# quadram-institute-bioscience/tatajuba

Measured on AMD Instinct MI355X. Metric: reads/s (whole node), 150 bp synthetic FASTQ, homopolymer scan + context histogram, higher is better.
Workload: dtype u8/u64

## Files before the change

tatajuba_amd/csrc/hopo_device.hip:

```cpp

#include <hip/hip_runtime.h>
#include <rccl/rccl.h>
#include <dlfcn.h>
#include <mutex>
#include <string>
#include <new>
#include <stdint.h>
#include <stdio.h>
#include <stdlib.h>
#include <string.h>
#include <stdarg.h>
#include <limits.h>
#include <float.h>
#include <algorithm>
#include <vector>
#include <memory>

#include "../../include/tatajuba_amd.h"
#include "../../include/tatajuba_variants.h"
#include "../../include/tatajuba_features.h"
#include "../../include/tatajuba_effects.h"
#include "../../include/tatajuba_sites.h"
#include "../../include/tatajuba_depths.h"
#include "../../include/tatajuba_distances.h"
// ... 1267 lines not shown
__device__ __noinline__ u64 fast_general_tract (const FastLds &T, const uint8_t *__restrict__ seq, long n_bytes, long g0, int s, int k, int mprime, bool n_tile)
{
  u64 c0, c1; u32 base, len10, flag;
  if (!fast_tract<true> (T, seq, n_bytes, g0, s, k, mprime, c0, c1, base, len10, flag, n_tile)) return 0ull;
  return pack_rec1 ((u32) c0, (u32) c1, base, len10, flag);
}

__device__ __forceinline__ void lds_dma32 (const uint8_t *sbase, u32 voff, void *lds_wave_base)
{
  const u32 m0v = (u32) (size_t) (lptr_t) lds_wave_base;
  asm volatile ("s_nop 0\n\tglobal_load_lds_dwordx4 %0, %1\n\tglobal_load_lds_dwordx4 %0, %1 offset:1024"
                :: "v"(voff), "s"(sbase), "{m0}"(m0v) : "memory");
}

template <int W, bool LOG = false>
__global__ __launch_bounds__ (FK_BLOCK, FK_BLOCK * (LOG ? FK_LOG_WG_PER_CU : FK_WG_PER_CU) / 256)
void scan_fast_kernel (const uint8_t *__restrict__ seq, long n_bytes, long n_ftiles, int k, int mprime,
                       Buckets BK, DevCounters *ctr, u32 *__restrict__ slow_list, int par, int all_slow, LogSpace LG)
{
  static_assert (!LOG || W <= 2, "the record log holds one-word and two-word records");
  __shared__ FastLds T;
  __shared__ uint4 raw[FK_WIN / 16];
  __shared__ std::conditional_t<LOG, LogLds, StageLds<W, true>> SL;
  auto make_sink = [&] () {
    if constexpr (LOG) return LogSink<W> {SL, LG, ctr, k, 0u, 0u, 0u, 0u, 0ull};
    else return StageSink<W, FK_BLOCK, true> {SL, BK, ctr, k, 0u, 0u, 0u};
  };
  auto sink = make_sink ();
  sink.start ();

  const int tid = threadIdx.x, lane = tid & 63;
// ... 1313 lines not shown
__global__ __launch_bounds__ (256)
void bin_count_kernel (const u64 *__restrict__ in, long n, int k, int nbits, u32 *__restrict__ bins, uint4 *__restrict__ cov, long cov_vec, int grouped,
                       const FinPlan *__restrict__ plan = nullptr)
{
  if (plan) { if (!plan->ok) return; n = plan->n1; nbits = plan->nbits; cov_vec = plan->t / 2; }
  for (long i = (long) blockIdx.x * 256 + threadIdx.x; i < cov_vec; i += (long) gridDim.x * 256) cov[i] = make_uint4 (0, 0, 0, 0);
  for (long i0 = (long) blockIdx.x * 256; i0 < n; i0 += (long) gridDim.x * 256) {
    const long i = i0 + threadIdx.x;
    u32 bin = 0;
    if (i < n) { const u64 *p = in + 3 * i; bin = bin_of_record (p[0], p[1], p[2], k, nbits); }
    (void) bin_reserve (bins, bin, i < n, grouped);
  }
}

#define BS_MAXBINS (1 << BS_MAXBITS)
#define WGS_CHUNK  16384

#define WGS_PAD(i) ((i) + ((i) >> 5))
struct WgScanLds { u32 a[WGS_CHUNK + WGS_CHUNK / 32 + 1]; u32 wsum[16]; u32 vmax; };

__device__ __forceinline__ u32 wg_exclusive_scan (const u32 *__restrict__ in, int n_all, u32 *__restrict__ out, u32 *__restrict__ out2, WgScanLds &L, u32 &vmax)
{
  const int tid = threadIdx.x, lane = tid & 63, wave = tid >> 6;
  if (tid == 0) L.vmax = 0;
  u32 carry = 0;
  for (int base = 0; base < n_all; base += WGS_CHUNK) {
    const int n = min (WGS_CHUNK, n_all - base);
    const int per = (n + 1023) / 1024;
    for (int i = tid; i < n; i += 1024) L.a[WGS_PAD (i)] = in[base + i];
    __syncthreads ();
    u32 sum = 0, mx = 0;
    for (int j = 0; j < per; j++) { const int b = tid * per + j; if (b < n) { const u32 v = L.a[WGS_PAD (b)]; sum += v; mx = max (mx, v); } }
    const u32 incl = wave_inclusive_scan (sum);
    if (lane == 63) L.wsum[wave] = incl;
    for (int o = 32; o > 0; o >>= 1) mx = max (mx, (u32) __shfl_down ((int) mx, o));
    if (lane == 0 && mx) atomicMax (&L.vmax, mx);
    __syncthreads ();
    u32 run = carry + incl - sum, total = 0;
    for (int w = 0; w < 16; w++) { const u32 x = L.wsum[w]; if (w < wave) run += x; total += x; }
    for (int j = 0; j < per; j++) { const int b = tid * per + j; if (b < n) { const u32 v = L.a[WGS_PAD (b)]; L.a[WGS_PAD (b)] = run; run += v; } }
    __syncthreads ();
    for (int i = tid; i < n; i += 1024) { const u32 v = L.a[WGS_PAD (i)]; out[base + i] = v; if (out2) out2[base + i] = v; }
    carry += total;
    __syncthreads ();
  }
  vmax = L.vmax;
  return carry;
}

__global__ __launch_bounds__ (1024)
void bin_scan_kernel (u32 *__restrict__ bins, int nbins, u32 *__restrict__ binstart, u32 rank_max, FinCounts *fin, const FinPlan *__restrict__ plan = nullptr)
{
  __shared__ WgScanLds L;
  u32 vmax;
  if (plan) { if (!plan->ok) return; nbins = plan->nbins; }
  const u32 total = wg_exclusive_scan (bins, nbins, binstart, bins, L, vmax);
  if (threadIdx.x == 0) { binstart[nbins] = total; fin->sort_fallback = vmax > rank_max ? 1u : 0u; }
}

__global__ __launch_bounds__ (256)
void bin_scatter_kernel (const u64 *__restrict__ in, u64 *__restrict__ out, long n, int k, int nbits, u32 *__restrict__ cursors,
                         const FinPlan *__restrict__ plan = nullptr, uint4 *__restrict__ cov = nullptr)
{
  if (plan) { if (!plan->ok) return; n = plan->n1; nbits = plan->nbits; }
  if (cov) for (long i = (long) blockIdx.x * 256 + threadIdx.x; i < plan->t / 2; i += (long) gridDim.x * 256) cov[i] = make_uint4 (0, 0, 0, 0);
  for (long i = (long) blockIdx.x * 256 + threadIdx.x; i < n; i += (long) gridDim.x * 256) {
    const u64 *p = in + 3 * i;
    const u64 a = p[0], b = p[1], m = p[2];
    u64 *q = out + 3 * (u64) atomicAdd (&cursors[bin_of_record (a, b, m, k, nbits)], 1u);
    q[0] = a; q[1] = b; q[2] = m;
  }
}
// ... 183 lines not shown
  if ((threadIdx.x & 63) == 0) s_best[threadIdx.x >> 6] = best;
  __syncthreads ();
  if (threadIdx.x == 0) {
    for (int w = 1; w < (int) blockDim.x / 64; w++) best = max (best, s_best[w]);
    if (best != INT_MIN) atomicMax (result, best);
  }
}

__global__ __launch_bounds__ (256)
void cov_max_kernel (const u64 *__restrict__ tab, long t, int *result)
{
  __shared__ int s_best[4];
  cov_max_part (tab, t, result, s_best);
}

#define BSI_WAVES 1

template <int J>
__device__ __forceinline__ u32 lane_xor (u32 v, int lane)
{
  if constexpr (J == 1) return (u32) __builtin_amdgcn_update_dpp (0, (int) v, 0xB1, 0xF, 0xF, false);
  else if constexpr (J == 2) return (u32) __builtin_amdgcn_update_dpp (0, (int) v, 0x4E, 0xF, 0xF, false);
  else if constexpr (J == 4 || J == 8) {
    const u32 up = (u32) __builtin_amdgcn_update_dpp (0, (int) v, 0x100 + J, 0xF, 0xF, false);
    const u32 dn = (u32) __builtin_amdgcn_update_dpp (0, (int) v, 0x110 + J, 0xF, 0xF, false);
    return (lane & J) ? dn : up;
  }
  else if constexpr (J == 16) { const auto r = __builtin_amdgcn_permlane16_swap (v, v, false, false); return (lane & 16) ? r[0] : r[1]; }
  else { const auto r = __builtin_amdgcn_permlane32_swap (v, v, false, false); return (lane & 32) ? r[0] : r[1]; }
}

__global__ __launch_bounds__ (64 * BSI_WAVES)
void bin_sort_index_kernel (const u64 *__restrict__ in, u64 *__restrict__ out, const u32 *__restrict__ binstart, int nbins, const FinCounts *fin,
                            int min_coverage, u64 *__restrict__ cov_tab, int log2t,
                            u32 *__restrict__ binctx, u32 *__restrict__ tstart, u32 *__restrict__ tend, const FinPlan *__restrict__ plan = nullptr,
                            int cov_direct = 0)
{
  __shared__ alignas (16) u32 hd[BSI_WAVES][BS_RANK_MAX];
  __shared__ u32 sz[BSI_WAVES][BS_RANK_MAX];
  const int lane = threadIdx.x & 63, wave = threadIdx.x >> 6;
  const int bin0 = (int) blockIdx.x * BSI_WAVES + wave;
  u32 st0 = 0, en0 = 0;
  if (bin0 < nbins) { st0 = binstart[bin0]; en0 = binstart[bin0 + 1]; }
  if (plan) { if (!plan->ok) return; nbins = plan->nbins; log2t = plan->log2t; cov_direct = (int) plan->cov_direct; }
  if (fin->sort_fallback) return;
  u32 *H = hd[wave], *E = sz[wave];
  for (int bin = bin0; bin < nbins; bin += gridDim.x * BSI_WAVES) {
    const u32 st = (bin == bin0) ? st0 : binstart[bin], s = ((bin == bin0) ? en0 : binstart[bin + 1]) - st;
    if (s == 0) { if (lane == 0) binctx[bin] = 0; continue; }
    const u64 *R = in + 3 * (u64) st;
    u32 nkeep = 0;
    if (s <= 64u) {
      const bool valid = (u32) lane < s;
      u64 a0 = 0, a1 = 0, am = 0;
      if (valid) { a0 = R[3 * lane]; a1 = R[3 * lane + 1]; am = R[3 * lane + 2]; }
      const int w = meta_count (am);
      u64 cas_a = 0, cas_b = 0;
      if (!cov_direct && valid) cov_add2_issue ((u32) (a0 & 0x7FFFFFFFull), (u32) (a1 & 0x7FFFFFFFull), w, cov_tab, log2t, cas_a, cas_b);
      u32 kh = valid ? 2u | ((u32) am & 1u) : 0u;
      u32 kl = ((((u32) (am >> TJ_META_LEN_SHIFT) & 0x3FFu) ^ 0x200u) << 6) | (63u - (u32) lane);
      u32 x0 = (u32) a0, x1 = (u32) (a0 >> 32), y0 = (u32) a1, y1 = (u32) (a1 >> 32), m0 = (u32) am, m1 = (u32) (am >> 32);
      auto step = [&] (auto jc, int kk) {
        constexpr int J = decltype (jc)::value;
        const u32 ox0 = lane_xor<J> (x0, lane), ox1 = lane_xor<J> (x1, lane), oy0 = lane_xor<J> (y0, lane), oy1 = lane_xor<J> (y1, lane);
        const u32 om0 = lane_xor<J> (m0, lane), om1 = lane_xor<J> (m1, lane), okh = lane_xor<J> (kh, lane), okl = lane_xor<J> (kl, lane);
        const u64 mx = ((u64) x1 << 32) | x0, my = ((u64) y1 << 32) | y0, ox = ((u64) ox1 << 32) | ox0, oy = ((u64) oy1 << 32) | oy0;
        const bool mine_first = (kh > okh) | ((kh == okh) & ((mx > ox) | ((mx == ox) & ((my > oy) | ((my == oy) & (kl > okl))))));
        const bool want_first = ((lane & kk) == 0) == ((lane & J) == 0);
        const bool take = mine_first != want_first;
        x0 = take ? ox0 : x0; x1 = take ? ox1 : x1; y0 = take ? oy0 : y0; y1 = take ? oy1 : y1;
        m0 = take ? om0 : m0; m1 = take ? om1 : m1; kh = take ? okh : kh; kl = take ? okl : kl;
      };
#pragma unroll
// ... 20 lines not shown
      const u32 last_incl = (u32) __builtin_amdgcn_ds_bpermute ((int) ((next_head - 1u) << 2), (int) incl);
      const int depth = (int) (last_incl - (incl - (u32) cnt));
      const bool keep = head & (depth >= min_coverage);
      const u64 keeps = __ballot (keep);
      if (keep) {
        const u32 o = (u32) __popcll (keeps & ((1ull << lane) - 1ull));
        tstart[st + o] = st + (u32) lane;
        tend[st + o] = st + next_head;
      }
      nkeep = (u32) __popcll (keeps);
      if (cov_direct) {
        if (head) { cov_direct_add ((u32) (b0 & 0x7FFFFFFFull), depth, cov_tab); cov_direct_add ((u32) (b1 & 0x7FFFFFFFull), depth, cov_tab); }
      }
      else if (valid) {
        asm volatile ("" : "+v"(cas_a), "+v"(cas_b));
        cov_add2_finish ((u32) (a0 & 0x7FFFFFFFull), (u32) (a1 & 0x7FFFFFFFull), w, cov_tab, log2t, cas_a, cas_b);
      }
      if (lane == 0) binctx[bin] = nkeep;
      asm volatile ("s_waitcnt lgkmcnt(0)" ::: "memory");
      __builtin_amdgcn_wave_barrier ();
      continue;
    }
    for (u32 t0 = 0; t0 < s; t0 += 64) {
      const u32 t = t0 + lane;
      bool keep = false;
      if (t < s) {
        const u64 a0 = R[3 * t], a1 = R[3 * t + 1], am = R[3 * t + 2];
        u32 rank = 0, ctx_before = 0, ctx_size = 0;
        int depth = 0;
        const u32 abase = (u32) am & 1u, alen = ((u32) (am >> TJ_META_LEN_SHIFT) & 0x3FFu) ^ 0x200u;
        for (u32 j0 = 0; j0 < s; j0 += 4) {
// ... 41 lines not shown
          o += ((g.x & 0x80000000u) && (g.x & 0x7FFFFFFFu) < rank) ? 1u : 0u;
          o += (j + 1u < s && (g.y & 0x80000000u) && (g.y & 0x7FFFFFFFu) < rank) ? 1u : 0u;
          o += (j + 2u < s && (g.z & 0x80000000u) && (g.z & 0x7FFFFFFFu) < rank) ? 1u : 0u;
          o += (j + 3u < s && (g.w & 0x80000000u) && (g.w & 0x7FFFFFFFu) < rank) ? 1u : 0u;
        }
        tstart[st + o] = st + rank;
        tend[st + o] = st + rank + E[t];
      }
    }
    if (lane == 0) binctx[bin] = nkeep;
    asm volatile ("s_waitcnt lgkmcnt(0)" ::: "memory");
    __builtin_amdgcn_wave_barrier ();
  }
}

__global__ __launch_bounds__ (1024)
void bin_ctx_scan_kernel (const u32 *__restrict__ binctx, int nbins, u32 *__restrict__ binout, FinCounts *fin, const FinPlan *__restrict__ plan = nullptr)
{
  __shared__ WgScanLds L;
  u32 vmax;
  if (plan) { if (!plan->ok) return; nbins = plan->nbins; }
  const u32 total = wg_exclusive_scan (binctx, nbins, binout, nullptr, L, vmax);
  if (threadIdx.x == 0 && !fin->sort_fallback) { fin->n_idx = total; fin->coverage = INT_MIN; }
}

__global__ __launch_bounds__ (256)
void bin_ctx_write_kernel (const u32 *__restrict__ binstart, const u32 *__restrict__ binctx, const u32 *__restrict__ binout, int nbins,
                           const u32 *__restrict__ tstart, const u32 *__restrict__ tend, int *__restrict__ idx_initial, int *__restrict__ idx_final,
                           const u64 *__restrict__ cov_tab, long t, FinCounts *fin, const FinPlan *__restrict__ plan = nullptr)
{
  __shared__ int s_best[4];
  if (plan) { if (!plan->ok) return; nbins = plan->nbins; t = plan->t; }
  if (fin->sort_fallback) return;
  const int lane = threadIdx.x & 63, wave = threadIdx.x >> 6;
  for (int bin = blockIdx.x * 4 + wave; bin < nbins; bin += gridDim.x * 4) {
    const u32 cnt = binctx[bin], st = binstart[bin], o0 = binout[bin];
    for (u32 o = lane; o < cnt; o += 64) { idx_initial[o0 + o] = (int) tstart[st + o]; idx_final[o0 + o] = (int) tend[st + o]; }
  }
  cov_max_part (cov_tab, t, &fin->coverage, s_best);
}

#define MG_RANK_MAX 256
#define TJ_META_SAMPLE_SHIFT 52

__global__ __launch_bounds__ (256)
void merge_scatter_kernel (const u64 *__restrict__ in, u64 *__restrict__ out, long n, int k, int nbits, u32 *__restrict__ cursors,
                           const long *__restrict__ starts, int n_samples)
{
  for (long i0 = (long) blockIdx.x * 256; i0 < n; i0 += (long) gridDim.x * 256) {
    const long i = i0 + threadIdx.x;
    const bool active = i < n;
    u64 a = 0, b = 0, m = 0;
    int lo = 0;
    if (active) {
// ... 227 lines not shown
  u64 raw_bound = 0;
  long n_undefined = 0;
  double slack = 1.0;
  DevBuf alt, hist, flags, segid, headpos, keep, outpos, scan_tmp, kept, idx_i, idx_f, cov, bins, binstart, binctx, ovf, grp_jt, grp_hist, fine;
  u32 bin_rank_max = BS_RANK_MAX;
  FinCounts *d_fin = nullptr, *h_fin = nullptr;
  struct DevState *d_state = nullptr, *h_state = nullptr;
  void *h_kept = nullptr; size_t h_kept_cap = 0;
  bool bins_zeroed = false;
  bool fine_dirty = false;
  bool bins_counted = false;
  long n_kept = 0; int n_idx = 0, coverage = 0, status = -1;
  hipEvent_t ev_done = nullptr;
  hipEvent_t ev_agg = nullptr;
  hipStream_t order_stream = nullptr;
  FinCarry fin;
  hipEvent_t marks[8] = {nullptr, nullptr, nullptr, nullptr, nullptr, nullptr, nullptr, nullptr};
  unsigned mark_seq = 0;
  long last_scan_launches = 0;
  unsigned scan_seq = 0;
  size_t piece_target = TJ_SCAN_PIECE_TARGET;
  int scan_grid_cap = 0;
  int dist_blocks = 0;
  int link_small = 1;
  int groups_small = 1;
  int clades_small = 1;
  bool buckets_clean = false;
  long plan_mismatches = 0;
  bool ctr_clean = false;
};
// ... 51 lines not shown
  int commit (tjamd_counter *c)
  {
    if (n > 16) return set_err (TJAMD_ERR_STATE, "a scratch cut of %d pieces (16 at most)", n);
    const int rc = ensure (c->lc_work, used, c->stream);
    for (int i = 0; i < n && !rc; i++) piece[i].put (piece[i].at, (char *) c->lc_work.p + piece[i].offset);
    return rc;
  }
};

static int read_back (tjamd_counter *c, const char *fn, const void *d, void *h, size_t words)
{
  hipError_t e = hipGetLastError ();
  if (e == hipSuccess && words) e = hipMemcpyAsync (h, d, words * 4, hipMemcpyDeviceToHost, c->stream);
  if (e == hipSuccess) e = hipStreamSynchronize (c->stream);
  return e == hipSuccess ? TJAMD_OK : set_err (TJAMD_ERR_HIP, "%s: failed: %s", fn, hipGetErrorString (e));
}

extern "C" tjamd_counter *tjamd_counter_create (int device, int kmer_size)
{
  int n = tjamd_device_count ();
  if (n <= 0) { set_err (TJAMD_ERR_NO_DEVICE, "no HIP device visible: the homopolymer-tract engine needs an MI355X (no CPU fallback)"); return NULL; }
  if (device < 0 || device >= n) { set_err (TJAMD_ERR_ARG, "device %d out of range [0,%d)", device, n); return NULL; }
  if (kmer_size < 2 || kmer_size > 32) { set_err (TJAMD_ERR_ARG, "kmer_size %d outside [2,32] (reference clamp: src/main.c:184-185)", kmer_size); return NULL; }
  HIPCHK_NULL (hipSetDevice (device));
  std::unique_ptr<tjamd_counter, void (*) (tjamd_counter *)> made (new tjamd_counter (), tjamd_counter_destroy);
  tjamd_counter *const c = made.get ();
  c->device = device; c->k = kmer_size;
  c->W = (kmer_size <= 12) ? 1 : (kmer_size <= 28) ? 2 : 4;
  hipDeviceProp_t prop;
  HIPCHK_NULL (hipGetDeviceProperties (&prop, device));
  c->n_cu = prop.multiProcessorCount > 0 ? prop.multiProcessorCount : 256;
  const char *bm = getenv ("TATAJUBA_AMD_BIN_MAX");
  if (bm && atoi (bm) >= 1 && atoi (bm) <= BS_RANK_MAX) c->bin_rank_max = (u32) atoi (bm);
  const char *pc = getenv ("TATAJUBA_AMD_SCAN_PIECE");
  if (pc && atol (pc) >= 4096) c->piece_target = (size_t) atol (pc);
  const char *sk = getenv ("TATAJUBA_AMD_SINK");
  if (sk && !strcmp (sk, "fused")) c->log_mode = 0;
  if (sk && !strcmp (sk, "log")) c->log_mode = 2;
  const char *fm = getenv ("TATAJUBA_AMD_FAST");
  if (fm && atoi (fm) >= 0 && atoi (fm) <= 2) c->fast_mode = atoi (fm);
  const char *sg = getenv ("TATAJUBA_AMD_SCAN_GRID");
  if (sg && atoi (sg) >= 1) c->scan_grid_cap = atoi (sg);
  const char *db = getenv ("TATAJUBA_AMD_DISTANCE_BLOCKS");
  if (db && atoi (db) >= 1) c->dist_blocks = atoi (db);
  const char *ls = getenv ("TATAJUBA_AMD_LINKAGE_SMALL");
  if (ls && !strcmp (ls, "0")) c->link_small = 0;
  const char *gs = getenv ("TATAJUBA_AMD_GROUPS_SMALL");
  if (gs && !strcmp (gs, "0")) c->groups_small = 0;
  const char *cs = getenv ("TATAJUBA_AMD_CLADES_SMALL");
  if (cs && !strcmp (cs, "0")) c->clades_small = 0;
  const char *sl = getenv ("TATAJUBA_AMD_BUCKET_SLACK");
  if (sl && atof (sl) >= 1.0) c->slack = atof (sl);
  HIPCHK_NULL (hipStreamCreateWithFlags (&c->own_stream, hipStreamNonBlocking));
// ... 9 lines not shown
  HIPCHK_NULL (hipMemsetAsync (c->d_state, 0, sizeof (DevState), c->stream));
  HIPCHK_NULL (hipMemsetAsync (c->d_lctr, 0, sizeof (DevCounters), c->stream));
  for (StageTimer &t : c->timer) HIPCHK_NULL (t.create ());
  HIPCHK_NULL (hipEventCreate (&c->ev_p1));
  HIPCHK_NULL (hipEventCreateWithFlags (&c->ev_done, hipEventDisableTiming));
  HIPCHK_NULL (hipEventCreateWithFlags (&c->ev_agg, hipEventDisableTiming));
  HIPCHK_NULL (hipStreamSynchronize (c->stream));
  return made.release ();
}

extern "C" void tjamd_counter_destroy (tjamd_counter *c)
{
  if (!c) return;
  (void) hipSetDevice (c->device);
  if (c->stream) (void) hipStreamSynchronize (c->stream);
  DevBuf *all[] = {&c->log, &c->logmeta, &c->pool, &c->table, &c->stage, &c->fix, &c->loc, &c->prefix, &c->rawlist, &c->slow, &c->alt, &c->hist, &c->flags, &c->segid, &c->headpos,
                   &c->keep, &c->outpos, &c->scan_tmp, &c->kept, &c->idx_i, &c->idx_f, &c->cov, &c->bins, &c->binstart, &c->binctx, &c->ovf, &c->grp_jt, &c->grp_hist, &c->fine,
                   &c->ts_cov, &c->ts_aux, &c->ut_tot, &c->ut_lev, &c->ut_fb, &c->ut_slots, &c->lc_work};
  for (DevBuf *b : all) release (*b);
  for (hipEvent_t ev : c->marks) if (ev) (void) hipEventDestroy (ev);
  if (c->d_state) (void) hipFree (c->d_state);
  if (c->d_lctr) (void) hipFree (c->d_lctr);
  if (c->d_cursors) (void) hipFree (c->d_cursors);
  if (c->h_state) (void) hipHostFree (c->h_state);
  if (c->h_kept) (void) hipHostFree (c->h_kept);
  for (StageTimer &t : c->timer) t.destroy ();
  if (c->ev_p1) (void) hipEventDestroy (c->ev_p1);
  for (int i = 0; i < TJ_PIECE_EVENTS; i++) { if (c->ev_pa[i]) (void) hipEventDestroy (c->ev_pa[i]); if (c->ev_pb[i]) (void) hipEventDestroy (c->ev_pb[i]); }
  if (c->ev_done) (void) hipEventDestroy (c->ev_done);
  if (c->ev_agg) (void) hipEventDestroy (c->ev_agg);
  if (c->own_stream) (void) hipStreamDestroy (c->own_stream);
  delete c;
}

extern "C" int tjamd_counter_device (const tjamd_counter *c) { return c ? c->device : -1; }

extern "C" int tjamd_counter_set_stream (tjamd_counter *c, void *hip_stream)
{
  if (!c) return set_err (TJAMD_ERR_ARG, "null counter");
  HIPCHK (hipSetDevice (c->device));
  HIPCHK (hipStreamSynchronize (c->stream));
  c->stream = hip_stream ? (hipStream_t) hip_stream : c->own_stream;
  return TJAMD_OK;
}

extern "C" int tjamd_counter_set_order_stream (tjamd_counter *c, void *hip_stream)
{
  if (!c) return set_err (TJAMD_ERR_ARG, "null counter");
  HIPCHK (hipSetDevice (c->device));
  HIPCHK (hipStreamSynchronize (c->stream));
  if (c->order_stream) HIPCHK (hipStreamSynchronize (c->order_stream));
  c->order_stream = (hipStream_t) hip_stream;
  return TJAMD_OK;
}

static Buckets make_buckets (const tjamd_counter *c)
{
  Buckets B;
  B.pool = (u64 *) c->pool.p; B.table = (u32 *) c->table.p; B.cursors = c->d_cursors; B.pool_next = c->d_cursors + TJ_P * TJ_CSTRIDE;
  B.pool_chunks = c->pool_chunks; B.maxj = c->maxj; B.ch_shift = (u32) std::max (c->ch_shift, 0);
  return B;
}

static int clear_buckets (tjamd_counter *c, bool snapshot = false)
{
  if (!c->buckets_clean || snapshot) {
    const bool fused = snapshot && c->fine_dirty && c->bins.p != nullptr;
    hipLaunchKernelGGL (clear_buckets_kernel, dim3 (TJ_P), dim3 (256), 0, c->stream, c->d_cursors, c->d_ctr,
                        (u32 *) (c->maxj ? c->table.p : nullptr), c->maxj, c->ch_shift, c->d_fin, (u32 *) c->bins.p, c->bins.p ? BS_MAXBINS : 0,
// ... 550 lines not shown
  HIPCHK (hipMemsetAsync (c->cov.p, 0, (size_t) t * 8, c->stream));
  hipLaunchKernelGGL (set_int_kernel, dim3 (1), dim3 (1), 0, c->stream, &c->d_fin->coverage, INT_MIN);
  hipLaunchKernelGGL (cov_insert_kernel, dim3 (grid_for (2 * n1)), dim3 (256), 0, c->stream, kept, n1, ctab, log2t);
  HIPCHK (hipGetLastError ());
  hipLaunchKernelGGL (cov_max_kernel, dim3 (std::min<unsigned> (grid_for (t), 256u)), dim3 (256), 0, c->stream, (const u64 *) ctab, t, &c->d_fin->coverage);
  HIPCHK (hipGetLastError ());
  if ((rc = end_fin_interval (c, c->stream))) return rc;
  HIPCHK (hipMemcpyAsync (c->h_fin, c->d_fin, sizeof (FinCounts), hipMemcpyDeviceToHost, c->stream));
  HIPCHK (hipStreamSynchronize (c->stream));
  return TJAMD_OK;
}

static int finalise_binned (tjamd_counter *c, long n1, int min_coverage, long cap = 0, bool wait = true)
{
  const bool planned = n1 == 0;
  const bool aside = planned && !wait && c->order_stream != nullptr && c->order_stream != c->stream;
  const hipStream_t st = aside ? c->order_stream : c->stream;
  const FinPlan *plan = planned ? &c->d_state->plan : nullptr;
  if (planned) n1 = cap;
  const int nbits = bin_bits_for (n1, c->k);
  const int nbins = planned ? BS_MAXBINS : 1 << nbits;
  int cov_direct = 0;
  const int log2t = planned ? cov_table_bits (n1) : cov_plan_bits (n1, c->k, &cov_direct);
  const long t = 1l << log2t;
  const bool fused = planned && c->bins_counted;
  c->bins_counted = false;
  int rc = ensure (c->alt, (size_t) n1 * 24, c->stream);
  if (!rc && !c->bins.p) { rc = ensure (c->bins, (size_t) (BS_MAXBINS + 1) * 4, c->stream); c->bins_zeroed = false; }
  if (!rc) rc = ensure (c->binstart, (size_t) (nbins + 1) * 4, c->stream);
  if (!rc) rc = ensure (c->binctx, (size_t) nbins * 8, c->stream);
  if (!rc) rc = ensure (c->headpos, (size_t) n1 * 4, c->stream);
  if (!rc) rc = ensure (c->outpos, (size_t) n1 * 4, c->stream);
  if (!rc) rc = ensure (c->idx_i, (size_t) n1 * 4, c->stream);
  if (!rc) rc = ensure (c->idx_f, (size_t) n1 * 4, c->stream);
  if (!rc) rc = ensure (c->cov, (size_t) t * 8, c->stream);
  if (rc) return rc;
  u32 *bins = (u32 *) c->bins.p, *binstart = (u32 *) c->binstart.p, *binctx = (u32 *) c->binctx.p, *binout = binctx + nbins;
  u32 *tstart = (u32 *) c->headpos.p, *tend = (u32 *) c->outpos.p;
  u64 *ctab = (u64 *) c->cov.p;
  if (!fused && !c->bins_zeroed) HIPCHK (hipMemsetAsync (bins, 0, (size_t) BS_MAXBINS * 4, c->stream));
  c->bins_zeroed = false;
  if (aside) { HIPCHK (hipEventRecord (c->ev_agg, c->stream)); HIPCHK (hipStreamWaitEvent (st, c->ev_agg, 0)); }
  const unsigned g1 = planned ? std::min<unsigned> (grid_for (n1), 2048u) : grid_for (n1);
  if (!fused) hipLaunchKernelGGL (bin_count_kernel, dim3 (g1), dim3 (256), 0, st, (const u64 *) c->kept.p, n1, c->k, nbits, bins,
                                  (uint4 *) c->cov.p, (long) (t / 2), 0, plan);
  hipLaunchKernelGGL (bin_scan_kernel, dim3 (1), dim3 (1024), 0, st, bins, nbins, binstart, c->bin_rank_max, c->d_fin, plan);
  hipLaunchKernelGGL (bin_scatter_kernel, dim3 (g1), dim3 (256), 0, st, (const u64 *) c->kept.p, (u64 *) c->alt.p, n1, c->k, nbits, bins, plan,
                      fused ? (uint4 *) c->cov.p : (uint4 *) nullptr);
  hipLaunchKernelGGL (bin_sort_index_kernel, dim3 ((unsigned) std::min (nbins / BSI_WAVES + 1, 16384)), dim3 (64 * BSI_WAVES), 0, st,
                      (const u64 *) c->alt.p, (u64 *) c->kept.p, (const u32 *) binstart, nbins, (const FinCounts *) c->d_fin, min_coverage,
                      ctab, log2t, binctx, tstart, tend, plan, cov_direct);
  hipLaunchKernelGGL (bin_ctx_scan_kernel, dim3 (1), dim3 (1024), 0, st, (const u32 *) binctx, nbins, binout, c->d_fin, plan);
  hipLaunchKernelGGL (bin_ctx_write_kernel, dim3 (256), dim3 (256), 0, st, (const u32 *) binstart, (const u32 *) binctx, (const u32 *) binout, nbins,
                      (const u32 *) tstart, (const u32 *) tend, (int *) c->idx_i.p, (int *) c->idx_f.p, (const u64 *) ctab, t, c->d_fin, plan);
  HIPCHK (hipGetLastError ());
  if ((rc = end_fin_interval (c, st))) return rc;
  if (planned) HIPCHK (hipMemcpyAsync (c->h_state, c->d_state, sizeof (DevState), hipMemcpyDeviceToHost, st));
  else HIPCHK (hipMemcpyAsync (c->h_fin, c->d_fin, sizeof (FinCounts), hipMemcpyDeviceToHost, c->stream));
  if (wait) HIPCHK (hipStreamSynchronize (c->stream));
  else HIPCHK (hipEventRecord (c->ev_done, st));
  return TJAMD_OK;
}

static int finalise_queue (tjamd_counter *c, int remove_biased, int min_coverage, bool wait)
{
  if (!c) return set_err (TJAMD_ERR_ARG, "null counter");
  HIPCHK (hipSetDevice (c->device));
  FinCarry &f = c->fin;
  f = FinCarry {FIN_IDLE, remove_biased, min_coverage};
  c->n_kept = 0; c->n_idx = 0; c->coverage = 0; c->timer[T_FIN].timed = false;
  f.speculative = (c->raw_bound / 2 + 1) * 24 <= (8ull << 30);
  f.kept_cap = c->raw_bound / 2 + 1;
  int rc = TJAMD_OK;
  if (!f.speculative) {
    rc = sync_counters (c);
    if (rc) return rc;
    if (c->n_raw_known == 0) { f.state = FIN_SETTLED; return finalise_status (c, nullptr, 1); }
    if (c->n_raw_known >= (1l << 31)) return set_err (TJAMD_ERR_CAPACITY, "%ld raw records exceed the reference's int n_elem", c->n_raw_known);
    f.kept_cap = (u64) c->n_raw_known / 2 + 1;
  }

  rc = ensure (c->kept, (size_t) f.kept_cap * 24, c->stream);
  if (!rc) rc = ensure (c->ovf, c->pool.cap, c->stream);
  if (rc) return rc;
  HIPCHK (c->timer[T_FIN].begin (c->stream));
// ... 1239 lines not shown
  if (!rc && !c->bins.p) { rc = ensure (c->bins, (size_t) (BS_MAXBINS + 1) * 4, c->stream); c->bins_zeroed = false; }
  if (!rc) rc = ensure (c->binstart, (size_t) (BS_MAXBINS + 1) * 4, c->stream);
  if (!rc) rc = ensure (c->binctx, (size_t) BS_MAXBINS * 8, c->stream);
  if (!rc) rc = ensure (c->headpos, (size_t) n * 4, c->stream);
  if (!rc) rc = ensure (c->outpos, (size_t) n * 4, c->stream);
  if (rc) return -rc;
  if (hipMemcpyAsync (c->prefix.p, starts.data (), (size_t) (n_samples + 1) * 8, hipMemcpyHostToDevice, c->stream) != hipSuccess ||
      hipStreamSynchronize (c->stream) != hipSuccess) return -set_err (TJAMD_ERR_HIP, "copy failed");
  u32 *bins = (u32 *) c->bins.p, *binstart = (u32 *) c->binstart.p, *binctx = (u32 *) c->binctx.p, *binout = binctx + nbins;
  u32 *tpos = (u32 *) c->headpos.p, *ttot = (u32 *) c->outpos.p;
  if (!c->bins_zeroed && hipMemsetAsync (bins, 0, (size_t) BS_MAXBINS * 4, c->stream) != hipSuccess) return -set_err (TJAMD_ERR_HIP, "memset failed");
  c->bins_zeroed = false;
  Stage st (c, T_MERGE);
  st.begin ();
  hipLaunchKernelGGL (bin_count_kernel, dim3 (grid_for (n)), dim3 (256), 0, c->stream, (const u64 *) d_records, n, c->k, nbits, bins, (uint4 *) nullptr, 0l, 1);
  hipLaunchKernelGGL (bin_scan_kernel, dim3 (1), dim3 (1024), 0, c->stream, bins, nbins, binstart,
                      c->bin_rank_max < (u32) BS_RANK_MAX ? c->bin_rank_max : (u32) MG_RANK_MAX, c->d_fin);
  hipLaunchKernelGGL (merge_scatter_kernel, dim3 (grid_for (n)), dim3 (256), 0, c->stream, (const u64 *) d_records, (u64 *) c->alt.p, n, c->k, nbits, bins,
                      (const long *) c->prefix.p, n_samples);
  hipLaunchKernelGGL (bin_merge_kernel, dim3 ((unsigned) std::min (nbins, 16384)), dim3 (64), 0, c->stream, (const u64 *) c->alt.p, (const u32 *) binstart, nbins,
                      (const FinCounts *) c->d_fin, binctx, tpos, ttot);
  hipLaunchKernelGGL (bin_ctx_scan_kernel, dim3 (1), dim3 (1024), 0, c->stream, (const u32 *) binctx, nbins, binout, c->d_fin);
  hipLaunchKernelGGL (bin_merge_write_kernel, dim3 ((unsigned) std::min (nbins / 4 + 1, 4096)), dim3 (256), 0, c->stream, (const u64 *) c->alt.p, (const u32 *) binstart,
                      (const u32 *) binout, nbins, (const FinCounts *) c->d_fin, (const u32 *) tpos, (const u32 *) ttot, n_samples,
                      (u64 *) d_out_keys, (int *) d_out_counts, capacity);
  if (hipGetLastError () != hipSuccess) return -set_err (TJAMD_ERR_HIP, "merge launch failed");
  st.end ();
  st.done ();
  if (hipMemcpyAsync (c->h_fin, c->d_fin, sizeof (FinCounts), hipMemcpyDeviceToHost, c->stream) != hipSuccess ||
      hipStreamSynchronize (c->stream) != hipSuccess) return -set_err (TJAMD_ERR_HIP, "merge failed: %s", hipGetErrorString (hipGetLastError ()));
  if (c->h_fin->sort_fallback) return merge_samples_radix (c, d_records, n, n_samples, d_out_keys, d_out_counts, capacity);
  const long n_union = c->h_fin->n_idx;
  if (n_union > capacity) return -set_err (TJAMD_ERR_CAPACITY, "%ld union keys, caller capacity %ld", n_union, capacity);
  return n_union;
}

static long merge_samples_radix (tjamd_counter *c, const void *d_records, long n, int n_samples, void *d_out_keys, void *d_out_counts, long capacity)
// ... 3671 lines not shown
```

Baseline: 11.44 billion.

## Restructure finalise ordering: register-scan, split small/large bin sort, shared side stream

The workgroup scan moves from an LDS-staged 1024-thread loop to a 256-thread vectorised register scan, with a serial fallback for unaligned inputs. Bin sorting is split into two kernels: a 64-thread pass that handles bins of up to 64 records and queues larger bins into a list, and a second capped-grid pass that sorts only the listed bins with LDS. Register caps are added to the scan kernel and the ordering kernels, and the DPP lane exchange and coverage max reduction are rewritten. Finalisation can now run on a shared per-device side stream by default. Together these aim to cut finalisation and launch-side latency overlapping the scan, at the cost of possible register spills and extra complexity in stream lifetime handling.

```diff
diff --git a/tatajuba_amd/csrc/hopo_device.hip b/tatajuba_amd/csrc/hopo_device.hip
--- a/tatajuba_amd/csrc/hopo_device.hip
+++ b/tatajuba_amd/csrc/hopo_device.hip
@@ -1305,7 +1305,7 @@
 }
 
 template <int W, bool LOG = false>
-__global__ __launch_bounds__ (FK_BLOCK, FK_BLOCK * (LOG ? FK_LOG_WG_PER_CU : FK_WG_PER_CU) / 256)
+__global__ __launch_bounds__ (FK_BLOCK, FK_BLOCK * (LOG ? FK_LOG_WG_PER_CU : FK_WG_PER_CU) / 256) __attribute__ ((amdgpu_num_sgpr (88)))
 void scan_fast_kernel (const uint8_t *__restrict__ seq, long n_bytes, long n_ftiles, int k, int mprime,
                        Buckets BK, DevCounters *ctr, u32 *__restrict__ slow_list, int par, int all_slow, LogSpace LG)
 {
@@ -2649,48 +2649,75 @@
 }
 
 #define BS_MAXBINS (1 << BS_MAXBITS)
-#define WGS_CHUNK  16384
-
-#define WGS_PAD(i) ((i) + ((i) >> 5))
-struct WgScanLds { u32 a[WGS_CHUNK + WGS_CHUNK / 32 + 1]; u32 wsum[16]; u32 vmax; };
+#define WGS_THREADS 256
+#define WGS_WAVES  (WGS_THREADS / 64)
+#define WGS_PER    8
+#define WGS_CHUNK  (WGS_THREADS * WGS_PER)
+#define ORDER_REGS   __attribute__ ((amdgpu_num_vgpr (16)))
+#define ORDER_KERNEL __launch_bounds__ (256) ORDER_REGS
+
+struct WgScanLds { u32 wsum[2][WGS_WAVES]; u32 vmax; };
 
 __device__ __forceinline__ u32 wg_exclusive_scan (const u32 *__restrict__ in, int n_all, u32 *__restrict__ out, u32 *__restrict__ out2, WgScanLds &L, u32 &vmax)
 {
   const int tid = threadIdx.x, lane = tid & 63, wave = tid >> 6;
+  if ((((size_t) in | (size_t) out | (size_t) out2) & 15) != 0 || (n_all & 3) != 0) {
+    u32 run = 0, mx = 0;
+    if (tid == 0) {
+      for (int i = 0; i < n_all; i++) { const u32 v = in[i]; out[i] = run; if (out2) out2[i] = run; run += v; mx = max (mx, v); }
+      L.wsum[0][0] = run; L.vmax = mx;
+    }
+    __syncthreads ();
+    vmax = L.vmax;
+    return L.wsum[0][0];
+  }
   if (tid == 0) L.vmax = 0;
+  __syncthreads ();
   u32 carry = 0;
-  for (int base = 0; base < n_all; base += WGS_CHUNK) {
-    const int n = min (WGS_CHUNK, n_all - base);
-    const int per = (n + 1023) / 1024;
-    for (int i = tid; i < n; i += 1024) L.a[WGS_PAD (i)] = in[base + i];
-    __syncthreads ();
+  int par = 0;
+  for (int base = 0; base < n_all; base += WGS_CHUNK, par ^= 1) {
+    const int i0 = base + tid * WGS_PER;
+    uint4 v[WGS_PER / 4];
+#pragma unroll
+    for (int q = 0; q < WGS_PER / 4; q++) {
+      v[q] = make_uint4 (0, 0, 0, 0);
+      if (i0 + 4 * q < n_all) v[q] = *reinterpret_cast<const uint4 *> (in + i0 + 4 * q);
+    }
     u32 sum = 0, mx = 0;
-    for (int j = 0; j < per; j++) { const int b = tid * per + j; if (b < n) { const u32 v = L.a[WGS_PAD (b)]; sum += v; mx = max (mx, v); } }
+#pragma unroll
+    for (int q = 0; q < WGS_PER / 4; q++) { sum += v[q].x + v[q].y + v[q].z + v[q].w; mx = max (max (mx, max (v[q].x, v[q].y)), max (v[q].z, v[q].w)); }
     const u32 incl = wave_inclusive_scan (sum);
-    if (lane == 63) L.wsum[wave] = incl;
+    if (lane == 63) L.wsum[par][wave] = incl;
     for (int o = 32; o > 0; o >>= 1) mx = max (mx, (u32) __shfl_down ((int) mx, o));
     if (lane == 0 && mx) atomicMax (&L.vmax, mx);
     __syncthreads ();
     u32 run = carry + incl - sum, total = 0;
-    for (int w = 0; w < 16; w++) { const u32 x = L.wsum[w]; if (w < wave) run += x; total += x; }
-    for (int j = 0; j < per; j++) { const int b = tid * per + j; if (b < n) { const u32 v = L.a[WGS_PAD (b)]; L.a[WGS_PAD (b)] = run; run += v; } }
-    __syncthreads ();
-    for (int i = tid; i < n; i += 1024) { const u32 v = L.a[WGS_PAD (i)]; out[base + i] = v; if (out2) out2[base + i] = v; }
+    for (int w = 0; w < WGS_WAVES; w++) { const u32 x = L.wsum[par][w]; if (w < wave) run += x; total += x; }
+#pragma unroll
+    for (int q = 0; q < WGS_PER / 4; q++) {
+      uint4 o;
+      o.x = run; run += v[q].x; o.y = run; run += v[q].y; o.z = run; run += v[q].z; o.w = run; run += v[q].w;
+      if (i0 + 4 * q < n_all) {
+        *reinterpret_cast<uint4 *> (out + i0 + 4 * q) = o;
+        if (out2) *reinterpret_cast<uint4 *> (out2 + i0 + 4 * q) = o;
+      }
+    }
     carry += total;
-    __syncthreads ();
-  }
+  }
+  __syncthreads ();
   vmax = L.vmax;
   return carry;
 }
 
-__global__ __launch_bounds__ (1024)
-void bin_scan_kernel (u32 *__restrict__ bins, int nbins, u32 *__restrict__ binstart, u32 rank_max, FinCounts *fin, const FinPlan *__restrict__ plan = nullptr)
+__global__ ORDER_KERNEL
+void bin_scan_kernel (u32 *__restrict__ bins, int nbins, u32 *__restrict__ binstart, u32 rank_max, FinCounts *fin, const FinPlan *__restrict__ plan = nullptr,
+                      u32 *__restrict__ full = nullptr)
 {
   __shared__ WgScanLds L;
   u32 vmax;
   if (plan) { if (!plan->ok) return; nbins = plan->nbins; }
   const u32 total = wg_exclusive_scan (bins, nbins, binstart, bins, L, vmax);
-  if (threadIdx.x == 0) { binstart[nbins] = total; fin->sort_fallback = vmax > rank_max ? 1u : 0u; }
+  if (threadIdx.x == 0) { binstart[nbins] = total; fin->sort_fallback = vmax > rank_max ? 1u : 0u; if (full) full[0] = 0u; }
 }
 
 __global__ __launch_bounds__ (256)
@@ -2904,7 +2931,7 @@
   cov_max_part (tab, t, result, s_best);
 }
 
-#define BSI_WAVES 1
+#define BSF_GRID 1024
 
 template <int J>
 __device__ __forceinline__ u32 lane_xor (u32 v, int lane)
@@ -2912,41 +2939,44 @@
   if constexpr (J == 1) return (u32) __builtin_amdgcn_update_dpp (0, (int) v, 0xB1, 0xF, 0xF, false);
   else if constexpr (J == 2) return (u32) __builtin_amdgcn_update_dpp (0, (int) v, 0x4E, 0xF, 0xF, false);
   else if constexpr (J == 4 || J == 8) {
-    const u32 up = (u32) __builtin_amdgcn_update_dpp (0, (int) v, 0x100 + J, 0xF, 0xF, false);
-    const u32 dn = (u32) __builtin_amdgcn_update_dpp (0, (int) v, 0x110 + J, 0xF, 0xF, false);
-    return (lane & J) ? dn : up;
+    constexpr int lo = J == 4 ? 0x5 : 0x3;
+    const int up = __builtin_amdgcn_update_dpp (0, (int) v, 0x100 + J, 0xF, lo, false);
+    return (u32) __builtin_amdgcn_update_dpp (up, (int) v, 0x110 + J, 0xF, 0xF ^ lo, false);
   }
   else if constexpr (J == 16) { const auto r = __builtin_amdgcn_permlane16_swap (v, v, false, false); return (lane & 16) ? r[0] : r[1]; }
   else { const auto r = __builtin_amdgcn_permlane32_swap (v, v, false, false); return (lane & 32) ? r[0] : r[1]; }
 }
 
-__global__ __launch_bounds__ (64 * BSI_WAVES)
-void bin_sort_index_kernel (const u64 *__restrict__ in, u64 *__restrict__ out, const u32 *__restrict__ binstart, int nbins, const FinCounts *fin,
-                            int min_coverage, u64 *__restrict__ cov_tab, int log2t,
-                            u32 *__restrict__ binctx, u32 *__restrict__ tstart, u32 *__restrict__ tend, const FinPlan *__restrict__ plan = nullptr,
-                            int cov_direct = 0)
-{
-  __shared__ alignas (16) u32 hd[BSI_WAVES][BS_RANK_MAX];
-  __shared__ u32 sz[BSI_WAVES][BS_RANK_MAX];
-  const int lane = threadIdx.x & 63, wave = threadIdx.x >> 6;
-  const int bin0 = (int) blockIdx.x * BSI_WAVES + wave;
+template <bool FULL>
+__device__ __forceinline__ void bin_sort_index_bins (const u64 *__restrict__ in, u64 *__restrict__ out, const u32 *__restrict__ binstart, int nbins, const FinCounts *fin,
+                                                     int min_coverage, u64 *__restrict__ cov_tab, int log2t,
+                                                     u32 *__restrict__ binctx, u32 *__restrict__ tstart, u32 *__restrict__ tend, const FinPlan *__restrict__ plan,
+                                                     int cov_direct, u32 *__restrict__ full, u32 *H, u32 *E)
+{
+  const int lane = threadIdx.x & 63;
+  const int bin0 = (int) blockIdx.x;
   u32 st0 = 0, en0 = 0;
-  if (bin0 < nbins) { st0 = binstart[bin0]; en0 = binstart[bin0 + 1]; }
+  if (!FULL && bin0 < nbins) { st0 = binstart[bin0]; en0 = binstart[bin0 + 1]; }
   if (plan) { if (!plan->ok) return; nbins = plan->nbins; log2t = plan->log2t; cov_direct = (int) plan->cov_direct; }
   if (fin->sort_fallback) return;
-  u32 *H = hd[wave], *E = sz[wave];
-  for (int bin = bin0; bin < nbins; bin += gridDim.x * BSI_WAVES) {
-    const u32 st = (bin == bin0) ? st0 : binstart[bin], s = ((bin == bin0) ? en0 : binstart[bin + 1]) - st;
+  const u32 n_turns = FULL ? min (full[0], (u32) nbins) : (u32) nbins;
+  for (u32 turn = blockIdx.x; turn < n_turns; turn += gridDim.x) {
+    const int bin = FULL ? (int) full[1 + turn] : (int) turn;
+    const u32 st = (!FULL && bin == bin0) ? st0 : binstart[bin], s = ((!FULL && bin == bin0) ? en0 : binstart[bin + 1]) - st;
     if (s == 0) { if (lane == 0) binctx[bin] = 0; continue; }
     const u64 *R = in + 3 * (u64) st;
     u32 nkeep = 0;
-    if (s <= 64u) {
+    if constexpr (!FULL) {
+      if (s <= 64u) {
+      }
+      else { if (lane == 0) full[1u + atomicAdd (&full[0], 1u)] = (u32) bin; continue; }
       const bool valid = (u32) lane < s;
       u64 a0 = 0, a1 = 0, am = 0;
       if (valid) { a0 = R[3 * lane]; a1 = R[3 * lane + 1]; am = R[3 * lane + 2]; }
       const int w = meta_count (am);
+      const u32 ka = (u32) a0 & 0x7FFFFFFFu, kb = (u32) a1 & 0x7FFFFFFFu;
       u64 cas_a = 0, cas_b = 0;
-      if (!cov_direct && valid) cov_add2_issue ((u32) (a0 & 0x7FFFFFFFull), (u32) (a1 & 0x7FFFFFFFull), w, cov_tab, log2t, cas_a, cas_b);
+      if (!cov_direct && valid) cov_add2_issue (ka, kb, w, cov_tab, log2t, cas_a, cas_b);
       u32 kh = valid ? 2u | ((u32) am & 1u) : 0u;
       u32 kl = ((((u32) (am >> TJ_META_LEN_SHIFT) & 0x3FFu) ^ 0x200u) << 6) | (63u - (u32) lane);
       u32 x0 = (u32) a0, x1 = (u32) (a0 >> 32), y0 = (u32) a1, y1 = (u32) (a1 >> 32), m0 = (u32) am, m1 = (u32) (am >> 32);
@@ -2997,7 +3027,7 @@
       }
       else if (valid) {
         asm volatile ("" : "+v"(cas_a), "+v"(cas_b));
-        cov_add2_finish ((u32) (a0 & 0x7FFFFFFFull), (u32) (a1 & 0x7FFFFFFFull), w, cov_tab, log2t, cas_a, cas_b);
+        cov_add2_finish (ka, kb, w, cov_tab, log2t, cas_a, cas_b);
       }
       if (lane == 0) binctx[bin] = nkeep;
       asm volatile ("s_waitcnt lgkmcnt(0)" ::: "memory");
@@ -3069,7 +3099,27 @@
   }
 }
 
-__global__ __launch_bounds__ (1024)
+__global__ __launch_bounds__ (64) ORDER_REGS
+void bin_sort_index_kernel (const u64 *__restrict__ in, u64 *__restrict__ out, const u32 *__restrict__ binstart, int nbins, const FinCounts *fin,
+                            int min_coverage, u64 *__restrict__ cov_tab, int log2t,
+                            u32 *__restrict__ binctx, u32 *__restrict__ tstart, u32 *__restrict__ tend, u32 *__restrict__ full,
+                            const FinPlan *__restrict__ plan = nullptr, int cov_direct = 0)
+{
+  bin_sort_index_bins<false> (in, out, binstart, nbins, fin, min_coverage, cov_tab, log2t, binctx, tstart, tend, plan, cov_direct, full, nullptr, nullptr);
+}
+
+__global__ __launch_bounds__ (64) ORDER_REGS
+void bin_sort_full_kernel (const u64 *__restrict__ in, u64 *__restrict__ out, const u32 *__restrict__ binstart, int nbins, const FinCounts *fin,
+                           int min_coverage, u64 *__restrict__ cov_tab, int log2t,
+                           u32 *__restrict__ binctx, u32 *__restrict__ tstart, u32 *__restrict__ tend, u32 *__restrict__ full,
+                           const FinPlan *__restrict__ plan = nullptr, int cov_direct = 0)
+{
+  __shared__ alignas (16) u32 hd[BS_RANK_MAX];
+  __shared__ u32 sz[BS_RANK_MAX];
+  bin_sort_index_bins<true> (in, out, binstart, nbins, fin, min_coverage, cov_tab, log2t, binctx, tstart, tend, plan, cov_direct, full, hd, sz);
+}
+
+__global__ ORDER_KERNEL
 void bin_ctx_scan_kernel (const u32 *__restrict__ binctx, int nbins, u32 *__restrict__ binout, FinCounts *fin, const FinPlan *__restrict__ plan = nullptr)
 {
   __shared__ WgScanLds L;
@@ -3079,7 +3129,7 @@
   if (threadIdx.x == 0 && !fin->sort_fallback) { fin->n_idx = total; fin->coverage = INT_MIN; }
 }
 
-__global__ __launch_bounds__ (256)
+__global__ ORDER_KERNEL
 void bin_ctx_write_kernel (const u32 *__restrict__ binstart, const u32 *__restrict__ binctx, const u32 *__restrict__ binout, int nbins,
                            const u32 *__restrict__ tstart, const u32 *__restrict__ tend, int *__restrict__ idx_initial, int *__restrict__ idx_final,
                            const u64 *__restrict__ cov_tab, long t, FinCounts *fin, const FinPlan *__restrict__ plan = nullptr)
@@ -3090,9 +3140,25 @@
   const int lane = threadIdx.x & 63, wave = threadIdx.x >> 6;
   for (int bin = blockIdx.x * 4 + wave; bin < nbins; bin += gridDim.x * 4) {
     const u32 cnt = binctx[bin], st = binstart[bin], o0 = binout[bin];
+#pragma unroll 1
     for (u32 o = lane; o < cnt; o += 64) { idx_initial[o0 + o] = (int) tstart[st + o]; idx_final[o0 + o] = (int) tend[st + o]; }
   }
-  cov_max_part (cov_tab, t, &fin->coverage, s_best);
+  int best = INT_MIN;
+  const uint4 *tab2 = reinterpret_cast<const uint4 *> (cov_tab);
+  const u32 half = (u32) (t >> 1);
+#pragma unroll 2
+  for (u32 i = blockIdx.x * 256u + threadIdx.x; i < half; i += gridDim.x * 256u) {
+    const uint4 v = tab2[i];
+    if (v.y) best = max (best, (int) v.x);
+    if (v.w) best = max (best, (int) v.z);
+  }
+  for (int o = 32; o > 0; o >>= 1) best = max (best, __shfl_down (best, o));
+  if (lane == 0) s_best[wave] = best;
+  __syncthreads ();
+  if (threadIdx.x == 0) {
+    for (int w = 1; w < 4; w++) best = max (best, s_best[w]);
+    if (best != INT_MIN) atomicMax (&fin->coverage, best);
+  }
 }
 
 #define MG_RANK_MAX 256
@@ -3350,6 +3416,9 @@
   hipEvent_t ev_done = nullptr;
   hipEvent_t ev_agg = nullptr;
   hipStream_t order_stream = nullptr;
+  enum { ORDER_SIDE, ORDER_MAIN, ORDER_GIVEN } order_mode = ORDER_SIDE;
+  bool side_held = false;
+  unsigned order_path = 0;
   FinCarry fin;
   hipEvent_t marks[8] = {nullptr, nullptr, nullptr, nullptr, nullptr, nullptr, nullptr, nullptr};
   unsigned mark_seq = 0;
@@ -3431,6 +3500,31 @@
   if (e == hipSuccess && words) e = hipMemcpyAsync (h, d, words * 4, hipMemcpyDeviceToHost, c->stream);
   if (e == hipSuccess) e = hipStreamSynchronize (c->stream);
   return e == hipSuccess ? TJAMD_OK : set_err (TJAMD_ERR_HIP, "%s: failed: %s", fn, hipGetErrorString (e));
+}
+
+#define TJ_SIDE_DEVICES 64
+static std::mutex g_side_mutex;
+static struct { hipStream_t stream; int users; } g_side[TJ_SIDE_DEVICES];
+
+static hipStream_t side_stream_acquire (tjamd_counter *c)
+{
+  if (c->device < 0 || c->device >= TJ_SIDE_DEVICES) return nullptr;
+  std::lock_guard<std::mutex> lock (g_side_mutex);
+  auto &s = g_side[c->device];
+  if (!c->side_held) {
+    if (!s.stream && hipStreamCreateWithFlags (&s.stream, hipStreamNonBlocking) != hipSuccess) { s.stream = nullptr; (void) hipGetLastError (); return nullptr; }
+    s.users++; c->side_held = true;
+  }
+  return s.stream;
+}
+
+static void side_stream_release (tjamd_counter *c)
+{
+  if (!c->side_held) return;
+  std::lock_guard<std::mutex> lock (g_side_mutex);
+  auto &s = g_side[c->device];
+  c->side_held = false;
+  if (--s.users == 0 && s.stream) { (void) hipStreamSynchronize (s.stream); (void) hipStreamDestroy (s.stream); s.stream = nullptr; }
 }
 
 extern "C" tjamd_counter *tjamd_counter_create (int device, int kmer_size)
@@ -3454,6 +3548,8 @@
   const char *sk = getenv ("TATAJUBA_AMD_SINK");
   if (sk && !strcmp (sk, "fused")) c->log_mode = 0;
   if (sk && !strcmp (sk, "log")) c->log_mode = 2;
+  const char *om = getenv ("TATAJUBA_AMD_ORDER");
+  if (om && !strcmp (om, "main")) c->order_mode = tjamd_counter::ORDER_MAIN;
   const char *fm = getenv ("TATAJUBA_AMD_FAST");
   if (fm && atoi (fm) >= 0 && atoi (fm) <= 2) c->fast_mode = atoi (fm);
   const char *sg = getenv ("TATAJUBA_AMD_SCAN_GRID");
@@ -3493,6 +3589,8 @@
   if (!c) return;
   (void) hipSetDevice (c->device);
   if (c->stream) (void) hipStreamSynchronize (c->stream);
+  if (c->fin.state == FIN_EVENT) (void) hipEventSynchronize (c->ev_done);
+  side_stream_release (c);
   DevBuf *all[] = {&c->log, &c->logmeta, &c->pool, &c->table, &c->stage, &c->fix, &c->loc, &c->prefix, &c->rawlist, &c->slow, &c->alt, &c->hist, &c->flags, &c->segid, &c->headpos,
                    &c->keep, &c->outpos, &c->scan_tmp, &c->kept, &c->idx_i, &c->idx_f, &c->cov, &c->bins, &c->binstart, &c->binctx, &c->ovf, &c->grp_jt, &c->grp_hist, &c->fine,
                    &c->ts_cov, &c->ts_aux, &c->ut_tot, &c->ut_lev, &c->ut_fb, &c->ut_slots, &c->lc_work};
@@ -3519,7 +3617,14 @@
   if (!c) return set_err (TJAMD_ERR_ARG, "null counter");
   HIPCHK (hipSetDevice (c->device));
   HIPCHK (hipStreamSynchronize (c->stream));
-  c->stream = hip_stream ? (hipStream_t) hip_stream : c->own_stream;
+  if (hip_stream) {
+    if (c->own_stream) { HIPCHK (hipStreamDestroy (c->own_stream)); c->own_stream = nullptr; }
+    c->stream = (hipStream_t) hip_stream;
+  }
+  else {
+    if (!c->own_stream) HIPCHK (hipStreamCreateWithFlags (&c->own_stream, hipStreamNonBlocking));
+    c->stream = c->own_stream;
+  }
   return TJAMD_OK;
 }
 
@@ -3528,10 +3633,13 @@
   if (!c) return set_err (TJAMD_ERR_ARG, "null counter");
   HIPCHK (hipSetDevice (c->device));
   HIPCHK (hipStreamSynchronize (c->stream));
-  if (c->order_stream) HIPCHK (hipStreamSynchronize (c->order_stream));
+  if (c->fin.state == FIN_EVENT) HIPCHK (hipEventSynchronize (c->ev_done));
   c->order_stream = (hipStream_t) hip_stream;
+  c->order_mode = tjamd_counter::ORDER_GIVEN;
   return TJAMD_OK;
 }
+
+extern "C" long tjamd_debug_order_path (tjamd_counter *c) { return c ? (long) c->order_path : -1; }
 
 static Buckets make_buckets (const tjamd_counter *c)
 {
@@ -4112,8 +4220,11 @@
 static int finalise_binned (tjamd_counter *c, long n1, int min_coverage, long cap = 0, bool wait = true)
 {
   const bool planned = n1 == 0;
-  const bool aside = planned && !wait && c->order_stream != nullptr && c->order_stream != c->stream;
-  const hipStream_t st = aside ? c->order_stream : c->stream;
+  hipStream_t other = nullptr;
+  if (planned && !wait) other = c->order_mode == tjamd_counter::ORDER_GIVEN ? c->order_stream : c->order_mode == tjamd_counter::ORDER_SIDE ? side_stream_acquire (c) : nullptr;
+  const bool aside = other != nullptr && other != c->stream;
+  const hipStream_t st = aside ? other : c->stream;
+  c->order_path |= aside ? 1u : planned ? 4u : 2u;
   const FinPlan *plan = planned ? &c->d_state->plan : nullptr;
   if (planned) n1 = cap;
   const int nbits = bin_bits_for (n1, c->k);
@@ -4126,14 +4237,14 @@
   int rc = ensure (c->alt, (size_t) n1 * 24, c->stream);
   if (!rc && !c->bins.p) { rc = ensure (c->bins, (size_t) (BS_MAXBINS + 1) * 4, c->stream); c->bins_zeroed = false; }
   if (!rc) rc = ensure (c->binstart, (size_t) (nbins + 1) * 4, c->stream);
-  if (!rc) rc = ensure (c->binctx, (size_t) nbins * 8, c->stream);
+  if (!rc) rc = ensure (c->binctx, ((size_t) nbins * 3 + 1) * 4, c->stream);
   if (!rc) rc = ensure (c->headpos, (size_t) n1 * 4, c->stream);
   if (!rc) rc = ensure (c->outpos, (size_t) n1 * 4, c->stream);
   if (!rc) rc = ensure (c->idx_i, (size_t) n1 * 4, c->stream);
   if (!rc) rc = ensure (c->idx_f, (size_t) n1 * 4, c->stream);
   if (!rc) rc = ensure (c->cov, (size_t) t * 8, c->stream);
   if (rc) return rc;
-  u32 *bins = (u32 *) c->bins.p, *binstart = (u32 *) c->binstart.p, *binctx = (u32 *) c->binctx.p, *binout = binctx + nbins;
+  u32 *bins = (u32 *) c->bins.p, *binstart = (u32 *) c->binstart.p, *binctx = (u32 *) c->binctx.p, *binout = binctx + nbins, *full = binout + nbins;
   u32 *tstart = (u32 *) c->headpos.p, *tend = (u32 *) c->outpos.p;
   u64 *ctab = (u64 *) c->cov.p;
   if (!fused && !c->bins_zeroed) HIPCHK (hipMemsetAsync (bins, 0, (size_t) BS_MAXBINS * 4, c->stream));
@@ -4142,13 +4253,16 @@
   const unsigned g1 = planned ? std::min<unsigned> (grid_for (n1), 2048u) : grid_for (n1);
   if (!fused) hipLaunchKernelGGL (bin_count_kernel, dim3 (g1), dim3 (256), 0, st, (const u64 *) c->kept.p, n1, c->k, nbits, bins,
                                   (uint4 *) c->cov.p, (long) (t / 2), 0, plan);
-  hipLaunchKernelGGL (bin_scan_kernel, dim3 (1), dim3 (1024), 0, st, bins, nbins, binstart, c->bin_rank_max, c->d_fin, plan);
+  hipLaunchKernelGGL (bin_scan_kernel, dim3 (1), dim3 (WGS_THREADS), 0, st, bins, nbins, binstart, c->bin_rank_max, c->d_fin, plan, full);
   hipLaunchKernelGGL (bin_scatter_kernel, dim3 (g1), dim3 (256), 0, st, (const u64 *) c->kept.p, (u64 *) c->alt.p, n1, c->k, nbits, bins, plan,
                       fused ? (uint4 *) c->cov.p : (uint4 *) nullptr);
-  hipLaunchKernelGGL (bin_sort_index_kernel, dim3 ((unsigned) std::min (nbins / BSI_WAVES + 1, 16384)), dim3 (64 * BSI_WAVES), 0, st,
+  hipLaunchKernelGGL (bin_sort_index_kernel, dim3 ((unsigned) std::min (nbins + 1, 16384)), dim3 (64), 0, st,
                       (const u64 *) c->alt.p, (u64 *) c->kept.p, (const u32 *) binstart, nbins, (const FinCounts *) c->d_fin, min_coverage,
-                      ctab, log2t, binctx, tstart, tend, plan, cov_direct);
-  hipLaunchKernelGGL (bin_ctx_scan_kernel, dim3 (1), dim3 (1024), 0, st, (const u32 *) binctx, nbins, binout, c->d_fin, plan);
+                      ctab, log2t, binctx, tstart, tend, full, plan, cov_direct);
+  hipLaunchKernelGGL (bin_sort_full_kernel, dim3 ((unsigned) std::min (nbins, BSF_GRID)), dim3 (64), 0, st,
+                      (const u64 *) c->alt.p, (u64 *) c->kept.p, (const u32 *) binstart, nbins, (const FinCounts *) c->d_fin, min_coverage,
+                      ctab, log2t, binctx, tstart, tend, full, plan, cov_direct);
+  hipLaunchKernelGGL (bin_ctx_scan_kernel, dim3 (1), dim3 (WGS_THREADS), 0, st, (const u32 *) binctx, nbins, binout, c->d_fin, plan);
   hipLaunchKernelGGL (bin_ctx_write_kernel, dim3 (256), dim3 (256), 0, st, (const u32 *) binstart, (const u32 *) binctx, (const u32 *) binout, nbins,
                       (const u32 *) tstart, (const u32 *) tend, (int *) c->idx_i.p, (int *) c->idx_f.p, (const u64 *) ctab, t, c->d_fin, plan);
   HIPCHK (hipGetLastError ());
@@ -4166,7 +4280,7 @@
   HIPCHK (hipSetDevice (c->device));
   FinCarry &f = c->fin;
   f = FinCarry {FIN_IDLE, remove_biased, min_coverage};
-  c->n_kept = 0; c->n_idx = 0; c->coverage = 0; c->timer[T_FIN].timed = false;
+  c->n_kept = 0; c->n_idx = 0; c->coverage = 0; c->timer[T_FIN].timed = false; c->order_path = 0;
   f.speculative = (c->raw_bound / 2 + 1) * 24 <= (8ull << 30);
   f.kept_cap = c->raw_bound / 2 + 1;
   int rc = TJAMD_OK;
@@ -5436,13 +5550,13 @@
   Stage st (c, T_MERGE);
   st.begin ();
   hipLaunchKernelGGL (bin_count_kernel, dim3 (grid_for (n)), dim3 (256), 0, c->stream, (const u64 *) d_records, n, c->k, nbits, bins, (uint4 *) nullptr, 0l, 1);
-  hipLaunchKernelGGL (bin_scan_kernel, dim3 (1), dim3 (1024), 0, c->stream, bins, nbins, binstart,
+  hipLaunchKernelGGL (bin_scan_kernel, dim3 (1), dim3 (WGS_THREADS), 0, c->stream, bins, nbins, binstart,
                       c->bin_rank_max < (u32) BS_RANK_MAX ? c->bin_rank_max : (u32) MG_RANK_MAX, c->d_fin);
   hipLaunchKernelGGL (merge_scatter_kernel, dim3 (grid_for (n)), dim3 (256), 0, c->stream, (const u64 *) d_records, (u64 *) c->alt.p, n, c->k, nbits, bins,
                       (const long *) c->prefix.p, n_samples);
   hipLaunchKernelGGL (bin_merge_kernel, dim3 ((unsigned) std::min (nbins, 16384)), dim3 (64), 0, c->stream, (const u64 *) c->alt.p, (const u32 *) binstart, nbins,
                       (const FinCounts *) c->d_fin, binctx, tpos, ttot);
-  hipLaunchKernelGGL (bin_ctx_scan_kernel, dim3 (1), dim3 (1024), 0, c->stream, (const u32 *) binctx, nbins, binout, c->d_fin);
+  hipLaunchKernelGGL (bin_ctx_scan_kernel, dim3 (1), dim3 (WGS_THREADS), 0, c->stream, (const u32 *) binctx, nbins, binout, c->d_fin);
   hipLaunchKernelGGL (bin_merge_write_kernel, dim3 ((unsigned) std::min (nbins / 4 + 1, 4096)), dim3 (256), 0, c->stream, (const u64 *) c->alt.p, (const u32 *) binstart,
                       (const u32 *) binout, nbins, (const FinCounts *) c->d_fin, (const u32 *) tpos, (const u32 *) ttot, n_samples,
                       (u64 *) d_out_keys, (int *) d_out_counts, capacity);
```

After: 12.03 billion, median of 6. 1.05x the previous value.
